# uclanlp/visualbert

Measured on NVIDIA H100. Metric: image-text pairs/sec fwd+bwd VisualBERT-base, higher is better.
Workload: dtype bf16

## Files before the change

### visualbert_b200/csrc/vb_attention.cuh

```cuda
#pragma once
#include <stdlib.h>

#include "../../include/vbert_b200.h"
#include "vb_common.cuh"

namespace vb {


constexpr int kHd = 64;
constexpr int kBlk = 64;
constexpr int kTileBytes = kBlk * kHd * 2;
constexpr float kLog2e = 1.4426950408889634f;

struct AttnParams {
    const bf16* qkv;
    const float* mask_bias;
    bf16* ctx;
    float* lse;
    const bf16* dctx;
    bf16* dqkv;
    float* drow;
    unsigned long long* keep;
    int B, S, A, H;
    float scale;
// ... 190 lines not shown
#pragma unroll
    for (int nt = 0; nt < 8; ++nt) m |= static_cast<unsigned long long>((bits16 >> (2 * nt)) & 3u) << (nt * 8 + 2 * t);
    m |= __shfl_xor_sync(0xffffffffu, m, 1);
    m |= __shfl_xor_sync(0xffffffffu, m, 2);
    return m;
}
__device__ __forceinline__ void store_acc(bf16* base, long long ld, int row0, int nrows, const float (&c)[8][4],
                                          int lane, float mul0, float mul1) {
    const int g = lane >> 2, t = lane & 3;
    const int ra = row0 + g, rb = row0 + g + 8;
#pragma unroll
    for (int nt = 0; nt < 8; ++nt) {
        const int col = nt * 8 + 2 * t;
        if (ra < nrows)
            *reinterpret_cast<uint32_t*>(base + static_cast<long long>(ra) * ld + col) =
                pack_bf16x2(c[nt][0] * mul0, c[nt][1] * mul0);
        if (rb < nrows)
            *reinterpret_cast<uint32_t*>(base + static_cast<long long>(rb) * ld + col) =
                pack_bf16x2(c[nt][2] * mul1, c[nt][3] * mul1);
    }
}


constexpr int kMaxSub = 4;

int attn_fwd_head(const AttnParams& p, int nkb, cudaStream_t st, bool mask_ready);
int attn_bwd_head(const AttnParams& p, int nkb, cudaStream_t st, bool delta_ready);
int attn_keep_mask(const AttnParams& p, int nkb, cudaStream_t st);
int attn_delta(const AttnParams& p, cudaStream_t st);
bool attn_wgmma_supported(const AttnParams& p);
int attn_fwd_wgmma(const AttnParams& p, cudaStream_t st, bool mask_ready);
int attn_bwd_wgmma(const AttnParams& p, cudaStream_t st, bool delta_ready);
int make_tmap_bf16(CUtensorMap* m, const void* ptr, uint64_t inner, uint64_t outer, uint64_t ld_elems, uint32_t box_outer);

}
```

### visualbert_b200/csrc/vb_attention_wgmma.cu

```cuda
#include "vb_attention.cuh"

namespace vb {

constexpr int kWgTile = kBlk * kHd * 2;
constexpr int kMaxWgmmaBlocks = 3;

template <int NKB>
struct AttnSmem {
    static constexpr int FWD_BYTES = 3 * NKB * kWgTile + NKB * kBlk * 4 + 16 + 1024;
    static constexpr int BWD_BYTES = (4 * NKB + NKB * NKB) * kWgTile + NKB * kBlk * 4 + 16 + 1024;
};

__device__ __forceinline__ uint64_t tile_desc(uint32_t saddr) { return wgmma_desc_sw128(saddr, kWgTile, 1024); }

__device__ __forceinline__ unsigned long long keep_word(const AttnParams& p, unsigned bh, int q, int kb, int nkb, int t) {
    if (p.drop_scale == 0.f) return ~0ull;
    return p.keep[(static_cast<unsigned long long>(bh) * (nkb * kBlk) + q) * nkb + kb] >> (2 * t);
}

template <int NKB>
__device__ __forceinline__ void qk_block(float (&s)[32], uint32_t sQ, uint32_t sK, int wg, int kb) {
#pragma unroll
    for (int k = 0; k < kHd / 16; ++k)
        wgmma_m64n64k16_ss<0, 0>(s, tile_desc(sQ + wg * kWgTile + k * 32), tile_desc(sK + kb * kWgTile + k * 32), k > 0 ? 1u : 0u);
}
__device__ __forceinline__ void pack_afrag(uint32_t (&a)[4], const float (&x)[32], int kk) {
    a[0] = pack_bf16x2(x[8 * kk], x[8 * kk + 1]);
    a[1] = pack_bf16x2(x[8 * kk + 2], x[8 * kk + 3]);
    a[2] = pack_bf16x2(x[8 * kk + 4], x[8 * kk + 5]);
    a[3] = pack_bf16x2(x[8 * kk + 6], x[8 * kk + 7]);
}
__device__ __forceinline__ void store_rows(bf16* base, long long ld, int r0, int nrows, const float (&x)[32], int t, float mul0, float mul1) {
#pragma unroll
    for (int j = 0; j < 8; ++j) {
        const int col = 8 * j + 2 * t;
        if (r0 < nrows) *reinterpret_cast<uint32_t*>(base + static_cast<long long>(r0) * ld + col) = pack_bf16x2(x[4 * j] * mul0, x[4 * j + 1] * mul0);
        if (r0 + 8 < nrows)
            *reinterpret_cast<uint32_t*>(base + static_cast<long long>(r0 + 8) * ld + col) = pack_bf16x2(x[4 * j + 2] * mul1, x[4 * j + 3] * mul1);
    }
}
__device__ __forceinline__ void store_tile(uint32_t tile, int r, const float (&x)[32], int t) {
#pragma unroll
    for (int j = 0; j < 8; ++j) {
        st_shared_u32(tile + swz(r, j) + 4 * t, pack_bf16x2(x[4 * j], x[4 * j + 1]));
        st_shared_u32(tile + swz(r + 8, j) + 4 * t, pack_bf16x2(x[4 * j + 2], x[4 * j + 3]));
    }
}

template <int NKB>
__global__ void __launch_bounds__(NKB * 128, 1)
attn_fwd_wgmma_kernel(const __grid_constant__ CUtensorMap tmQKV, const AttnParams p) {
    extern __shared__ uint8_t smem_raw[];
    const uint32_t raw = smem_u32(smem_raw);
    const uint32_t base = (raw + 1023u) & ~1023u;
    uint8_t* smem = smem_raw + (base - raw);
    const uint32_t sQ = base, sK = base + NKB * kWgTile, sV = base + 2 * NKB * kWgTile;
    float* sbias = reinterpret_cast<float*>(smem + 3 * NKB * kWgTile);
    const uint32_t bar = base + 3 * NKB * kWgTile + NKB * kBlk * 4;
    const int tid = threadIdx.x, wg = tid >> 7, warp = (tid >> 5) & 3, lane = tid & 31, g = lane >> 2, t = lane & 3;
    const int item = blockIdx.x, b = item / p.A, h = item % p.A, S = p.S;
    const unsigned bh = static_cast<unsigned>(item);

    if (tid == 0) {
        tma_prefetch_desc(&tmQKV);
        mbar_init(bar, 1);
        fence_barrier_init();
    }
    __syncthreads();
    pdl_trigger();
    pdl_wait();
    if (tid == 0) {
        mbar_arrive_expect_tx(bar, 3 * NKB * kWgTile);
#pragma unroll
        for (int m = 0; m < 3; ++m)
#pragma unroll
            for (int kb = 0; kb < NKB; ++kb) tma_load_2d(base + (m * NKB + kb) * kWgTile, &tmQKV, bar, m * p.H + h * kHd, b * S + kb * kBlk);
    }
    for (int i = tid; i < NKB * kBlk; i += NKB * 128) sbias[i] = i < S ? p.mask_bias[static_cast<long long>(b) * S + i] * kLog2e : -INFINITY;
    const int q0 = wg * kBlk + warp * 16 + g;
    unsigned long long keep[NKB][2];
#pragma unroll
    for (int kb = 0; kb < NKB; ++kb) {
        keep[kb][0] = keep_word(p, bh, q0, kb, NKB, t);
        keep[kb][1] = keep_word(p, bh, q0 + 8, kb, NKB, t);
    }
    __syncthreads();
    mbar_wait(bar, 0);

    float s[NKB][32];
    wgmma_fence();
#pragma unroll
    for (int kb = 0; kb < NKB; ++kb) qk_block<NKB>(s[kb], sQ, sK, wg, kb);
    wgmma_commit();
    wgmma_wait<0>();

    const float sc2 = p.scale * kLog2e;
    float mx[2] = {-INFINITY, -INFINITY};
#pragma unroll
    for (int kb = 0; kb < NKB; ++kb)
#pragma unroll
        for (int j = 0; j < 8; ++j) {
            const float b0 = sbias[kb * kBlk + 8 * j + 2 * t], b1 = sbias[kb * kBlk + 8 * j + 2 * t + 1];
            s[kb][4 * j] = fmaf(s[kb][4 * j], sc2, b0); s[kb][4 * j + 1] = fmaf(s[kb][4 * j + 1], sc2, b1);
            s[kb][4 * j + 2] = fmaf(s[kb][4 * j + 2], sc2, b0); s[kb][4 * j + 3] = fmaf(s[kb][4 * j + 3], sc2, b1);
            mx[0] = fmaxf(mx[0], fmaxf(s[kb][4 * j], s[kb][4 * j + 1]));
            mx[1] = fmaxf(mx[1], fmaxf(s[kb][4 * j + 2], s[kb][4 * j + 3]));
        }
    float l[2] = {0.f, 0.f};
#pragma unroll
    for (int r = 0; r < 2; ++r) {
        mx[r] = fmaxf(mx[r], __shfl_xor_sync(0xffffffffu, mx[r], 1));
        mx[r] = fmaxf(mx[r], __shfl_xor_sync(0xffffffffu, mx[r], 2));
    }
#pragma unroll
    for (int kb = 0; kb < NKB; ++kb)
#pragma unroll
        for (int j = 0; j < 8; ++j)
#pragma unroll
            for (int c = 0; c < 4; ++c) {
                const int r = c >> 1;
                float e = fast_ex2(s[kb][4 * j + c] - mx[r]);
                l[r] += e;
                if (!((keep[kb][r] >> (8 * j + (c & 1))) & 1ull)) e = 0.f;
                s[kb][4 * j + c] = e;
            }
#pragma unroll
    for (int r = 0; r < 2; ++r) {
        l[r] += __shfl_xor_sync(0xffffffffu, l[r], 1);
        l[r] += __shfl_xor_sync(0xffffffffu, l[r], 2);
    }

    uint32_t pa[NKB][4][4];
#pragma unroll
    for (int kb = 0; kb < NKB; ++kb)
#pragma unroll
        for (int kk = 0; kk < 4; ++kk) pack_afrag(pa[kb][kk], s[kb], kk);
    float o[32];
    wgmma_fence();
#pragma unroll
    for (int kb = 0; kb < NKB; ++kb)
#pragma unroll
        for (int kk = 0; kk < 4; ++kk)
            wgmma_m64n64k16_rs<1>(o, pa[kb][kk], tile_desc(sV + kb * kWgTile + kk * 2048), (kb > 0 || kk > 0) ? 1u : 0u);
    wgmma_commit();
    wgmma_wait<0>();

    const float dscale = p.drop_scale != 0.f ? p.drop_scale : 1.f;
    store_rows(p.ctx + static_cast<long long>(b) * S * p.H + h * kHd, p.H, q0, S, o, t, dscale / l[0], dscale / l[1]);
    if (t == 0 && p.lse != nullptr) {
        float* lse = p.lse + static_cast<long long>(item) * S;
        if (q0 < S) lse[q0] = (mx[0] + log2f(l[0])) * 0.6931471805599453f;
        if (q0 + 8 < S) lse[q0 + 8] = (mx[1] + log2f(l[1])) * 0.6931471805599453f;
    }
}

template <int NKB>
__global__ void __launch_bounds__(NKB * 128, 1)
attn_bwd_wgmma_kernel(const __grid_constant__ CUtensorMap tmQKV, const __grid_constant__ CUtensorMap tmDO, const AttnParams p) {
    extern __shared__ uint8_t smem_raw[];
    const uint32_t raw = smem_u32(smem_raw);
    const uint32_t base = (raw + 1023u) & ~1023u;
    uint8_t* smem = smem_raw + (base - raw);
    const uint32_t sQ = base, sK = base + NKB * kWgTile, sV = base + 2 * NKB * kWgTile, sDO = base + 3 * NKB * kWgTile;
    const uint32_t sPS = base + 4 * NKB * kWgTile;
    float* sbias = reinterpret_cast<float*>(smem + (4 * NKB + NKB * NKB) * kWgTile);
    const uint32_t bar = base + (4 * NKB + NKB * NKB) * kWgTile + NKB * kBlk * 4;
    const int tid = threadIdx.x, wg = tid >> 7, warp = (tid >> 5) & 3, lane = tid & 31, g = lane >> 2, t = lane & 3;
    const int item = blockIdx.x, b = item / p.A, h = item % p.A, S = p.S;
    const unsigned bh = static_cast<unsigned>(item);
    const long long ld = 3LL * p.H;

    if (tid == 0) {
        tma_prefetch_desc(&tmQKV);
        tma_prefetch_desc(&tmDO);
        mbar_init(bar, 1);
        fence_barrier_init();
    }
    __syncthreads();
    pdl_trigger();
    pdl_wait();
    if (tid == 0) {
        mbar_arrive_expect_tx(bar, 4 * NKB * kWgTile);
#pragma unroll
        for (int kb = 0; kb < NKB; ++kb) {
#pragma unroll
            for (int m = 0; m < 3; ++m) tma_load_2d(base + (m * NKB + kb) * kWgTile, &tmQKV, bar, m * p.H + h * kHd, b * S + kb * kBlk);
            tma_load_2d(sDO + kb * kWgTile, &tmDO, bar, h * kHd, b * S + kb * kBlk);
        }
    }
    for (int i = tid; i < NKB * kBlk; i += NKB * 128) sbias[i] = i < S ? p.mask_bias[static_cast<long long>(b) * S + i] * kLog2e : -INFINITY;
    const int r0 = warp * 16 + g;
    const int q0 = wg * kBlk + r0;
    float lse2[2], dr[2];
#pragma unroll
    for (int r = 0; r < 2; ++r) {
        const int q = q0 + 8 * r;
        lse2[r] = q < S ? p.lse[static_cast<long long>(item) * S + q] * kLog2e : INFINITY;
        dr[r] = q < S ? p.drow[static_cast<long long>(item) * S + q] : 0.f;
    }
    unsigned long long keep[NKB][2];
#pragma unroll
    for (int kb = 0; kb < NKB; ++kb) {
        keep[kb][0] = keep_word(p, bh, q0, kb, NKB, t);
        keep[kb][1] = keep_word(p, bh, q0 + 8, kb, NKB, t);
    }
    __syncthreads();
    mbar_wait(bar, 0);
    const float sc2 = p.scale * kLog2e;
    const float ds = p.drop_scale != 0.f ? p.drop_scale : 1.f;
    auto probs = [&](float (&s)[32], int kb) {
#pragma unroll
        for (int j = 0; j < 8; ++j)
#pragma unroll
            for (int c = 0; c < 4; ++c)
                s[4 * j + c] = fast_ex2(fmaf(s[4 * j + c], sc2, sbias[kb * kBlk + 8 * j + 2 * t + (c & 1)]) - lse2[c >> 1]);
    };
    auto kept = [&](int kb, int j, int c) { return ((keep[kb][c >> 1] >> (8 * j + (c & 1))) & 1ull) != 0; };
    bf16* dqkv = p.dqkv + static_cast<long long>(b) * S * ld + h * kHd;

#pragma unroll
    for (int kb = 0; kb < NKB; ++kb) {
        float s[32];
        wgmma_fence();
        qk_block<NKB>(s, sQ, sK, wg, kb);
        wgmma_commit();
        wgmma_wait<0>();
        probs(s, kb);
#pragma unroll
        for (int j = 0; j < 8; ++j)
#pragma unroll
            for (int c = 0; c < 4; ++c) s[4 * j + c] = kept(kb, j, c) ? s[4 * j + c] * ds : 0.f;
        store_tile(sPS + (wg * NKB + kb) * kWgTile, r0, s, t);
    }
    fence_proxy_async_smem();
    __syncthreads();
    {
        float acc[32];
        wgmma_fence();
#pragma unroll
        for (int qb = 0; qb < NKB; ++qb)
#pragma unroll
            for (int kk = 0; kk < 4; ++kk)
                wgmma_m64n64k16_ss<1, 1>(acc, tile_desc(sPS + (qb * NKB + wg) * kWgTile + kk * 2048), tile_desc(sDO + qb * kWgTile + kk * 2048),
                                         (qb > 0 || kk > 0) ? 1u : 0u);
        wgmma_commit();
        wgmma_wait<0>();
        store_rows(dqkv + 2 * p.H, ld, q0, S, acc, t, 1.f, 1.f);
    }
    __syncthreads();

    float dq[32];
#pragma unroll
    for (int kb = 0; kb < NKB; ++kb) {
        float s[32], dp[32];
        wgmma_fence();
        qk_block<NKB>(s, sQ, sK, wg, kb);
#pragma unroll
        for (int k = 0; k < kHd / 16; ++k)
            wgmma_m64n64k16_ss<0, 0>(dp, tile_desc(sDO + wg * kWgTile + k * 32), tile_desc(sV + kb * kWgTile + k * 32), k > 0 ? 1u : 0u);
        wgmma_commit();
        wgmma_wait<0>();
        probs(s, kb);
#pragma unroll
        for (int j = 0; j < 8; ++j)
#pragma unroll
            for (int c = 0; c < 4; ++c) {
                const float dpd = kept(kb, j, c) ? dp[4 * j + c] * ds : 0.f;
                s[4 * j + c] *= dpd - dr[c >> 1];
            }
        store_tile(sPS + (wg * NKB + kb) * kWgTile, r0, s, t);
        uint32_t pa[4][4];
#pragma unroll
        for (int kk = 0; kk < 4; ++kk) pack_afrag(pa[kk], s, kk);
        wgmma_fence();
#pragma unroll
        for (int kk = 0; kk < 4; ++kk)
            wgmma_m64n64k16_rs<1>(dq, pa[kk], tile_desc(sK + kb * kWgTile + kk * 2048), (kb > 0 || kk > 0) ? 1u : 0u);
        wgmma_commit();
        wgmma_wait<0>();
    }
    store_rows(dqkv, ld, q0, S, dq, t, p.scale, p.scale);
    fence_proxy_async_smem();
    __syncthreads();
    {
        float acc[32];
        wgmma_fence();
#pragma unroll
        for (int qb = 0; qb < NKB; ++qb)
#pragma unroll
            for (int kk = 0; kk < 4; ++kk)
                wgmma_m64n64k16_ss<1, 1>(acc, tile_desc(sPS + (qb * NKB + wg) * kWgTile + kk * 2048), tile_desc(sQ + qb * kWgTile + kk * 2048),
                                         (qb > 0 || kk > 0) ? 1u : 0u);
        wgmma_commit();
        wgmma_wait<0>();
        store_rows(dqkv + p.H, ld, q0, S, acc, t, p.scale, p.scale);
    }
}

bool attn_wgmma_supported(const AttnParams& p) {
    return p.S <= kMaxWgmmaBlocks * kBlk && (reinterpret_cast<uintptr_t>(p.qkv) & 15) == 0 && (p.H * 2) % 16 == 0 &&
           (p.dctx == nullptr || (reinterpret_cast<uintptr_t>(p.dctx) & 15) == 0);
}

template <int NKB>
static int launch_fwd_wgmma(const AttnParams& p, const CUtensorMap& tq, cudaStream_t st) {
    auto kern = attn_fwd_wgmma_kernel<NKB>;
    static int configured[kMaxDevices] = {0};
    VB_CHECK_CUDA(ensure_dyn_smem(kern, AttnSmem<NKB>::FWD_BYTES, configured));
    ProfScope ps(st, PROF_ATTN_FWD, 4.0 * p.B * p.A * p.S * p.S * kHd, 1);
    VB_CHECK_CUDA(launch_pdl(kern, dim3(p.B * p.A), dim3(NKB * 128), AttnSmem<NKB>::FWD_BYTES, st, tq, p));
    return 0;
}
template <int NKB>
static int launch_bwd_wgmma(const AttnParams& p, const CUtensorMap& tq, const CUtensorMap& td, cudaStream_t st) {
    auto kern = attn_bwd_wgmma_kernel<NKB>;
    static int configured[kMaxDevices] = {0};
    VB_CHECK_CUDA(ensure_dyn_smem(kern, AttnSmem<NKB>::BWD_BYTES, configured));
    ProfScope ps(st, PROF_ATTN_DKV, 10.0 * p.B * p.A * p.S * p.S * kHd, 1);
    VB_CHECK_CUDA(launch_pdl(kern, dim3(p.B * p.A), dim3(NKB * 128), AttnSmem<NKB>::BWD_BYTES, st, tq, td, p));
    return 0;
}

int attn_fwd_wgmma(const AttnParams& p, cudaStream_t st, bool mask_ready) {
    const int nkb = (p.S + kBlk - 1) / kBlk;
    if (!mask_ready) {
        int rc = attn_keep_mask(p, nkb, st);
        if (rc) return rc;
    }
    CUtensorMap tq;
    int rc = make_tmap_bf16(&tq, p.qkv, 3ull * p.H, static_cast<uint64_t>(p.B) * p.S, 3ull * p.H, kBlk);
    if (rc) return rc;
    if (nkb == 1) rc = launch_fwd_wgmma<1>(p, tq, st);
    else if (nkb == 2) rc = launch_fwd_wgmma<2>(p, tq, st);
    else rc = launch_fwd_wgmma<3>(p, tq, st);
    if (rc) return rc;
    VB_CHECK_CUDA(cudaGetLastError());
    return 0;
}

int attn_bwd_wgmma(const AttnParams& p, cudaStream_t st, bool delta_ready) {
    const int nkb = (p.S + kBlk - 1) / kBlk;
    int rc = 0;
    if (!delta_ready) {
        rc = attn_delta(p, st);
        if (rc) return rc;
    }
    CUtensorMap tq, td;
    rc = make_tmap_bf16(&tq, p.qkv, 3ull * p.H, static_cast<uint64_t>(p.B) * p.S, 3ull * p.H, kBlk);
    if (rc) return rc;
    rc = make_tmap_bf16(&td, p.dctx, static_cast<uint64_t>(p.H), static_cast<uint64_t>(p.B) * p.S, static_cast<uint64_t>(p.H), kBlk);
    if (rc) return rc;
    if (nkb == 1) rc = launch_bwd_wgmma<1>(p, tq, td, st);
    else if (nkb == 2) rc = launch_bwd_wgmma<2>(p, tq, td, st);
    else rc = launch_bwd_wgmma<3>(p, tq, td, st);
    if (rc) return rc;
    VB_CHECK_CUDA(cudaGetLastError());
    return 0;
}

}
```

### visualbert_b200/csrc/vb_common.cuh

```cuda
#pragma once

#include <cuda.h>
#include <cuda_bf16.h>
#include <cuda_runtime.h>
#include <stdint.h>
#include <stdio.h>

#include <atomic>

namespace vb {

typedef __nv_bfloat16 bf16;

extern std::atomic<long long> g_launches;
int num_sms();
constexpr int kMaxDevices = 64;
int current_device();
template <typename K>
inline cudaError_t ensure_dyn_smem(K kern, int bytes, int (&cache)[kMaxDevices]) {
    const int d = current_device();
    if (cache[d] >= bytes) return cudaSuccess;
    cudaError_t e = cudaFuncSetAttribute(kern, cudaFuncAttributeMaxDynamicSharedMemorySize, bytes);
    if (e == cudaSuccess) cache[d] = bytes;
    return e;
// ... 156 lines not shown
__device__ __forceinline__ bool mbar_try_wait(uint32_t bar, uint32_t parity) {
    uint32_t ok;
    asm volatile(
        "{\n"
        ".reg .pred p;\n"
        "mbarrier.try_wait.parity.shared::cta.b64 p, [%1], %2;\n"
        "selp.u32 %0, 1, 0, p;\n"
        "}\n"
        : "=r"(ok)
        : "r"(bar), "r"(parity)
        : "memory");
    return ok != 0;
}
__device__ __forceinline__ void mbar_wait(uint32_t bar, uint32_t parity) {
    if (mbar_try_wait(bar, parity)) return;
    const long long t0 = clock64();
    uint32_t spins = 0;
    while (!mbar_try_wait(bar, parity)) {
        if ((++spins & 0x3ffu) == 0 && clock64() - t0 > 4000000000ll) __trap();
    }
}

__device__ __forceinline__ void tma_prefetch_desc(const CUtensorMap* m) {
    asm volatile("prefetch.tensormap [%0];" ::"l"(reinterpret_cast<uint64_t>(m)) : "memory");
}
__device__ __forceinline__ void tma_load_2d(uint32_t smem_dst, const CUtensorMap* m, uint32_t bar,
                                            int c_inner, int c_outer) {
    asm volatile(
        "cp.async.bulk.tensor.2d.shared::cluster.global.mbarrier::complete_tx::bytes"
        " [%0], [%1, {%3, %4}], [%2];"
        ::"r"(smem_dst), "l"(reinterpret_cast<uint64_t>(m)), "r"(bar), "r"(c_inner), "r"(c_outer)
        : "memory");
}

__device__ __forceinline__ uint64_t wgmma_desc_sw128(uint32_t saddr, uint32_t lbo_bytes, uint32_t sbo_bytes) {
    return static_cast<uint64_t>((saddr & 0x3FFFFu) >> 4) | (static_cast<uint64_t>((lbo_bytes >> 4) & 0x3FFFu) << 16) |
           (static_cast<uint64_t>((sbo_bytes >> 4) & 0x3FFFu) << 32) | (1ull << 62);
}
__device__ __forceinline__ void wgmma_fence() { asm volatile("wgmma.fence.sync.aligned;" ::: "memory"); }
__device__ __forceinline__ void wgmma_commit() { asm volatile("wgmma.commit_group.sync.aligned;" ::: "memory"); }
template <int N>
__device__ __forceinline__ void wgmma_wait() { asm volatile("wgmma.wait_group.sync.aligned %0;" ::"n"(N) : "memory"); }
template <int TA, int TB>
__device__ __forceinline__ void wgmma_m64n128k16(float (&d)[64], uint64_t a_desc, uint64_t b_desc, uint32_t accumulate) {
    asm volatile(
        "{\n"
        ".reg .pred p;\n"
        "setp.ne.b32 p, %66, 0;\n"
        "wgmma.mma_async.sync.aligned.m64n128k16.f32.bf16.bf16 "
        "{%0, %1, %2, %3, %4, %5, %6, %7, %8, %9, %10, %11, %12, %13, %14, %15, %16, %17, %18, %19, %20, %21, %22, %23, %24, %25, %26, %27, %28, %29, %30, %31, %32, %33, %34, %35, %36, %37, %38, %39, %40, %41, %42, %43, %44, %45, %46, %47, %48, %49, %50, %51, %52, %53, %54, %55, %56, %57, %58, %59, %60, %61, %62, %63}, "
        "%64, %65, p, 1, 1, %67, %68;\n"
        "}\n"
        : "+f"(d[0]), "+f"(d[1]), "+f"(d[2]), "+f"(d[3]), "+f"(d[4]), "+f"(d[5]), "+f"(d[6]), "+f"(d[7]),
          "+f"(d[8]), "+f"(d[9]), "+f"(d[10]), "+f"(d[11]), "+f"(d[12]), "+f"(d[13]), "+f"(d[14]), "+f"(d[15]),
          "+f"(d[16]), "+f"(d[17]), "+f"(d[18]), "+f"(d[19]), "+f"(d[20]), "+f"(d[21]), "+f"(d[22]), "+f"(d[23]),
          "+f"(d[24]), "+f"(d[25]), "+f"(d[26]), "+f"(d[27]), "+f"(d[28]), "+f"(d[29]), "+f"(d[30]), "+f"(d[31]),
          "+f"(d[32]), "+f"(d[33]), "+f"(d[34]), "+f"(d[35]), "+f"(d[36]), "+f"(d[37]), "+f"(d[38]), "+f"(d[39]),
          "+f"(d[40]), "+f"(d[41]), "+f"(d[42]), "+f"(d[43]), "+f"(d[44]), "+f"(d[45]), "+f"(d[46]), "+f"(d[47]),
          "+f"(d[48]), "+f"(d[49]), "+f"(d[50]), "+f"(d[51]), "+f"(d[52]), "+f"(d[53]), "+f"(d[54]), "+f"(d[55]),
          "+f"(d[56]), "+f"(d[57]), "+f"(d[58]), "+f"(d[59]), "+f"(d[60]), "+f"(d[61]), "+f"(d[62]), "+f"(d[63])
        : "l"(a_desc), "l"(b_desc), "r"(accumulate), "n"(TA), "n"(TB));
}
template <int TA, int TB>
__device__ __forceinline__ void wgmma_m64n64k16_ss(float (&d)[32], uint64_t a_desc, uint64_t b_desc, uint32_t accumulate) {
    asm volatile(
        "{\n"
// ... 67 lines not shown
```

### visualbert_b200/csrc/vb_gemm.cu

```cuda
#include <stdarg.h>
#include <stdio.h>
#include <stdlib.h>
#include <string.h>

#include <atomic>
#include <mutex>
#include <vector>

#include "../../include/vbert_b200.h"
#include "vb_common.cuh"

namespace vb {

static thread_local char g_err[1024] = "";
std::atomic<long long> g_launches{0};

void set_error(const char* fmt, ...) {
    va_list ap;
    va_start(ap, fmt);
    vsnprintf(g_err, sizeof(g_err), fmt, ap);
    va_end(ap);
}
const char* get_error() { return g_err; }

// ... 399 lines not shown
                              const cuuint32_t* box) {
    TmapKey k;
    memset(&k, 0, sizeof(k));
    k.ptr = ptr; k.rank = rank; k.dev = current_device();
    k.d0 = dims[0]; k.d1 = dims[1]; k.d2 = rank > 2 ? dims[2] : 1;
    k.s0 = strides[0]; k.s1 = rank > 2 ? strides[1] : 0;
    k.b0 = box[0]; k.b1 = box[1]; k.b2 = rank > 2 ? box[2] : 1;
    uint64_t h = reinterpret_cast<uintptr_t>(ptr) * 0x9E3779B97F4A7C15ull;
    h ^= (k.d0 * 31 + k.d1) * 0xBF58476D1CE4E5B9ull + k.d2 * 1315423911ull + k.s0 * 2654435761ull + k.s1 * 40503ull;
    h ^= (static_cast<uint64_t>(k.b1) << 20) ^ (static_cast<uint64_t>(k.b0) << 8) ^ k.b2 ^ (static_cast<uint64_t>(k.dev) << 40);
    h ^= h >> 29;
    if (g_tmap_cache == nullptr) { g_tmap_cache = new std::vector<TmapSlot>(kTmapSlots); for (auto& sl : *g_tmap_cache) sl.used = false; }
    TmapSlot& sl = (*g_tmap_cache)[h & (kTmapSlots - 1)];
    if (sl.used && sl.key == k) { *m = sl.map; return 0; }
    EncodeTiledFn fn = get_encode_fn();
    VB_REQUIRE(fn != nullptr, "cuTensorMapEncodeTiled unavailable (driver too old / no GPU?)");
    cuuint32_t estr[3] = {1, 1, 1};
    CUresult r = fn(m, CU_TENSOR_MAP_DATA_TYPE_BFLOAT16, rank, const_cast<void*>(ptr), dims, strides, box, estr,
                    CU_TENSOR_MAP_INTERLEAVE_NONE, CU_TENSOR_MAP_SWIZZLE_128B, CU_TENSOR_MAP_L2_PROMOTION_L2_256B,
                    CU_TENSOR_MAP_FLOAT_OOB_FILL_NONE);
    VB_REQUIRE(r == CUDA_SUCCESS, "cuTensorMapEncodeTiled (rank %u) failed with CUresult %d", rank, static_cast<int>(r));
    sl.key = k; sl.map = *m; sl.used = true;
    return 0;
}

int make_tmap_bf16(CUtensorMap* m, const void* ptr, uint64_t inner, uint64_t outer, uint64_t ld_elems,
                   uint32_t box_outer) {
    VB_REQUIRE((reinterpret_cast<uintptr_t>(ptr) & 15) == 0, "TMA operand not 16-byte aligned");
    VB_REQUIRE((ld_elems * 2) % 16 == 0, "TMA operand row stride must be a multiple of 8 elements");
    cuuint64_t dims[2] = {inner, outer};
    cuuint64_t strides[1] = {ld_elems * 2};
    cuuint32_t box[2] = {64, box_outer};
    return encode_tmap_cached(m, ptr, 2, dims, strides, box);
}

int current_device() {
    int dev = 0;
    cudaGetDevice(&dev);
    return (dev < 0 || dev >= kMaxDevices) ? 0 : dev;
}

int num_sms() {
    static int n[kMaxDevices] = {0};
    const int dev = current_device();
    if (n[dev] == 0) {
        int v = 0;
        cudaDeviceGetAttribute(&v, cudaDevAttrMultiProcessorCount, dev);
        n[dev] = v > 0 ? v : 132;
    }
    return n[dev];
}

template <bool A_MN, bool B_MN, int BLOCK_N, bool OUT_F32, int EPI = EPI_GENERIC>
static int launch(const CUtensorMap& ta, const CUtensorMap& tb, const GemmParams& p, cudaStream_t st) {
    using C = Cfg<BLOCK_N>;
    auto kern = gemm_wgmma_kernel<A_MN, B_MN, BLOCK_N, OUT_F32, EPI>;
    static int configured[kMaxDevices] = {0};
    VB_CHECK_CUDA(ensure_dyn_smem(kern, C::SMEM_BYTES, configured));
    const long long tiles = static_cast<long long>((p.M + BLOCK_M - 1) / BLOCK_M) * ((p.N + BLOCK_N - 1) / BLOCK_N) * p.splits;
    VB_REQUIRE(tiles < (1LL << 31), "vb_gemm: too many tiles");
    {
        ProfScope ps(st, OUT_F32 ? PROF_GEMM_WGRAD : (B_MN ? PROF_GEMM_DGRAD : PROF_GEMM_FWD), 2.0 * p.M * p.N * p.K, 1);
        VB_CHECK_CUDA(launch_pdl(kern, dim3(static_cast<unsigned>(tiles)), dim3(kThreads), C::SMEM_BYTES, st, ta, tb, p));
    }
    VB_CHECK_CUDA(cudaGetLastError());
    return 0;
// ... 167 lines not shown
```

Measured before the change: 3029.

## Make attention fwd/bwd kernels persistent with double-buffered TMA prefetch of next head

Attention forward and backward kernels become persistent: the grid is capped at SMs times occupancy and each block loops over (batch, head) items. While the current item computes, the next item's Q/K/V (forward) or Q/dO (backward) tiles are prefetched into a second shared-memory stage, along with its bias, LSE and dropout words. K/V in backward are reloaded after their last use. A 3D tensor map (inner, rows, batch) replaces the 2D one, so out-of-range rows are zero-filled per batch instead of reading into the next sequence. The cost is double the shared memory for staging, which may lower occupancy or block larger NKB configs.

Result: no change. 3042 (median of 6 runs) (+0.4%).

```diff
diff --git a/visualbert_b200/csrc/vb_attention.cuh b/visualbert_b200/csrc/vb_attention.cuh
--- a/visualbert_b200/csrc/vb_attention.cuh
+++ b/visualbert_b200/csrc/vb_attention.cuh
@@ -246,5 +246,7 @@
 int attn_fwd_wgmma(const AttnParams& p, cudaStream_t st, bool mask_ready);
 int attn_bwd_wgmma(const AttnParams& p, cudaStream_t st, bool delta_ready);
 int make_tmap_bf16(CUtensorMap* m, const void* ptr, uint64_t inner, uint64_t outer, uint64_t ld_elems, uint32_t box_outer);
-
-}
+int make_tmap_bf16_3d(CUtensorMap* m, const void* ptr, uint64_t inner, uint64_t rows, uint64_t batches, uint64_t ld_elems,
+                      uint32_t box_rows);
+
+}
diff --git a/visualbert_b200/csrc/vb_attention_wgmma.cu b/visualbert_b200/csrc/vb_attention_wgmma.cu
--- a/visualbert_b200/csrc/vb_attention_wgmma.cu
+++ b/visualbert_b200/csrc/vb_attention_wgmma.cu
@@ -7,8 +7,8 @@
 
 template <int NKB>
 struct AttnSmem {
-    static constexpr int FWD_BYTES = 3 * NKB * kWgTile + NKB * kBlk * 4 + 16 + 1024;
-    static constexpr int BWD_BYTES = (4 * NKB + NKB * NKB) * kWgTile + NKB * kBlk * 4 + 16 + 1024;
+    static constexpr int FWD_BYTES = 2 * 3 * NKB * kWgTile + 2 * NKB * kBlk * 4 + 16 + 1024;
+    static constexpr int BWD_BYTES = (6 * NKB + NKB * NKB) * kWgTile + NKB * kBlk * 4 + 32 + 1024;
 };
 
 __device__ __forceinline__ uint64_t tile_desc(uint32_t saddr) { return wgmma_desc_sw128(saddr, kWgTile, 1024); }
@@ -46,111 +46,131 @@
         st_shared_u32(tile + swz(r + 8, j) + 4 * t, pack_bf16x2(x[4 * j + 2], x[4 * j + 3]));
     }
 }
+template <int NKB>
+__device__ __forceinline__ void load_bias(float* sbias, const AttnParams& p, int b, int tid) {
+    for (int i = tid; i < NKB * kBlk; i += NKB * 128) sbias[i] = i < p.S ? p.mask_bias[static_cast<long long>(b) * p.S + i] * kLog2e : -INFINITY;
+}
 
 template <int NKB>
 __global__ void __launch_bounds__(NKB * 128, 1)
 attn_fwd_wgmma_kernel(const __grid_constant__ CUtensorMap tmQKV, const AttnParams p) {
+    constexpr int kStage = 3 * NKB * kWgTile;
     extern __shared__ uint8_t smem_raw[];
     const uint32_t raw = smem_u32(smem_raw);
     const uint32_t base = (raw + 1023u) & ~1023u;
     uint8_t* smem = smem_raw + (base - raw);
-    const uint32_t sQ = base, sK = base + NKB * kWgTile, sV = base + 2 * NKB * kWgTile;
-    float* sbias = reinterpret_cast<float*>(smem + 3 * NKB * kWgTile);
-    const uint32_t bar = base + 3 * NKB * kWgTile + NKB * kBlk * 4;
+    float* sbias0 = reinterpret_cast<float*>(smem + 2 * kStage);
+    const uint32_t bar0 = base + 2 * kStage + 2 * NKB * kBlk * 4;
     const int tid = threadIdx.x, wg = tid >> 7, warp = (tid >> 5) & 3, lane = tid & 31, g = lane >> 2, t = lane & 3;
-    const int item = blockIdx.x, b = item / p.A, h = item % p.A, S = p.S;
-    const unsigned bh = static_cast<unsigned>(item);
+    const int S = p.S, total = p.B * p.A;
+    const int q0 = wg * kBlk + warp * 16 + g;
+
+    auto load_item = [&](int it, int st) {
+        const int b = it / p.A, h = it % p.A;
+        const uint32_t bar = bar0 + 8 * st;
+        mbar_arrive_expect_tx(bar, kStage);
+#pragma unroll
+        for (int m = 0; m < 3; ++m)
+#pragma unroll
+            for (int kb = 0; kb < NKB; ++kb)
+                tma_load_3d(base + st * kStage + (m * NKB + kb) * kWgTile, &tmQKV, bar, m * p.H + (h * kHd), kb * kBlk, b);
+    };
+    unsigned long long keep[NKB][2];
+    auto read_item = [&](int it, int st) {
+        load_bias<NKB>(sbias0 + st * NKB * kBlk, p, it / p.A, tid);
+#pragma unroll
+        for (int kb = 0; kb < NKB; ++kb) {
+            keep[kb][0] = keep_word(p, static_cast<unsigned>(it), q0, kb, NKB, t);
+            keep[kb][1] = keep_word(p, static_cast<unsigned>(it), q0 + 8, kb, NKB, t);
+        }
+    };
 
     if (tid == 0) {
         tma_prefetch_desc(&tmQKV);
-        mbar_init(bar, 1);
+        mbar_init(bar0, 1);
+        mbar_init(bar0 + 8, 1);
         fence_barrier_init();
     }
     __syncthreads();
     pdl_trigger();
     pdl_wait();
-    if (tid == 0) {
-        mbar_arrive_expect_tx(bar, 3 * NKB * kWgTile);
-#pragma unroll
-        for (int m = 0; m < 3; ++m)
-#pragma unroll
-            for (int kb = 0; kb < NKB; ++kb) tma_load_2d(base + (m * NKB + kb) * kWgTile, &tmQKV, bar, m * p.H + h * kHd, b * S + kb * kBlk);
-    }
-    for (int i = tid; i < NKB * kBlk; i += NKB * 128) sbias[i] = i < S ? p.mask_bias[static_cast<long long>(b) * S + i] * kLog2e : -INFINITY;
-    const int q0 = wg * kBlk + warp * 16 + g;
-    unsigned long long keep[NKB][2];
-#pragma unroll
-    for (int kb = 0; kb < NKB; ++kb) {
-        keep[kb][0] = keep_word(p, bh, q0, kb, NKB, t);
-        keep[kb][1] = keep_word(p, bh, q0 + 8, kb, NKB, t);
-    }
-    __syncthreads();
-    mbar_wait(bar, 0);
-
-    float s[NKB][32];
-    wgmma_fence();
-#pragma unroll
-    for (int kb = 0; kb < NKB; ++kb) qk_block<NKB>(s[kb], sQ, sK, wg, kb);
-    wgmma_commit();
-    wgmma_wait<0>();
-
-    const float sc2 = p.scale * kLog2e;
-    float mx[2] = {-INFINITY, -INFINITY};
-#pragma unroll
-    for (int kb = 0; kb < NKB; ++kb)
-#pragma unroll
-        for (int j = 0; j < 8; ++j) {
-            const float b0 = sbias[kb * kBlk + 8 * j + 2 * t], b1 = sbias[kb * kBlk + 8 * j + 2 * t + 1];
-            s[kb][4 * j] = fmaf(s[kb][4 * j], sc2, b0); s[kb][4 * j + 1] = fmaf(s[kb][4 * j + 1], sc2, b1);
-            s[kb][4 * j + 2] = fmaf(s[kb][4 * j + 2], sc2, b0); s[kb][4 * j + 3] = fmaf(s[kb][4 * j + 3], sc2, b1);
-            mx[0] = fmaxf(mx[0], fmaxf(s[kb][4 * j], s[kb][4 * j + 1]));
-            mx[1] = fmaxf(mx[1], fmaxf(s[kb][4 * j + 2], s[kb][4 * j + 3]));
-        }
-    float l[2] = {0.f, 0.f};
-#pragma unroll
-    for (int r = 0; r < 2; ++r) {
-        mx[r] = fmaxf(mx[r], __shfl_xor_sync(0xffffffffu, mx[r], 1));
-        mx[r] = fmaxf(mx[r], __shfl_xor_sync(0xffffffffu, mx[r], 2));
-    }
-#pragma unroll
-    for (int kb = 0; kb < NKB; ++kb)
-#pragma unroll
-        for (int j = 0; j < 8; ++j)
-#pragma unroll
-            for (int c = 0; c < 4; ++c) {
-                const int r = c >> 1;
-                float e = fast_ex2(s[kb][4 * j + c] - mx[r]);
-                l[r] += e;
-                if (!((keep[kb][r] >> (8 * j + (c & 1))) & 1ull)) e = 0.f;
-                s[kb][4 * j + c] = e;
+    if (tid == 0) load_item(blockIdx.x, 0);
+    read_item(blockIdx.x, 0);
+
+    for (int item = blockIdx.x, i = 0; item < total; item += gridDim.x, ++i) {
+        const int st = i & 1, b = item / p.A, h = item % p.A, next = item + gridDim.x;
+        const uint32_t sQ = base + st * kStage, sK = sQ + NKB * kWgTile, sV = sQ + 2 * NKB * kWgTile;
+        const float* sbias = sbias0 + st * NKB * kBlk;
+        __syncthreads();
+        if (tid == 0 && next < total) load_item(next, st ^ 1);
+        mbar_wait(bar0 + 8 * st, (i >> 1) & 1);
+
+        float s[NKB][32];
+        wgmma_fence();
+#pragma unroll
+        for (int kb = 0; kb < NKB; ++kb) qk_block<NKB>(s[kb], sQ, sK, wg, kb);
+        wgmma_commit();
+        wgmma_wait<0>();
+
+        const float sc2 = p.scale * kLog2e;
+        float mx[2] = {-INFINITY, -INFINITY};
+#pragma unroll
+        for (int kb = 0; kb < NKB; ++kb)
+#pragma unroll
+            for (int j = 0; j < 8; ++j) {
+                const float b0 = sbias[kb * kBlk + 8 * j + 2 * t], b1 = sbias[kb * kBlk + 8 * j + 2 * t + 1];
+                s[kb][4 * j] = fmaf(s[kb][4 * j], sc2, b0); s[kb][4 * j + 1] = fmaf(s[kb][4 * j + 1], sc2, b1);
+                s[kb][4 * j + 2] = fmaf(s[kb][4 * j + 2], sc2, b0); s[kb][4 * j + 3] = fmaf(s[kb][4 * j + 3], sc2, b1);
+                mx[0] = fmaxf(mx[0], fmaxf(s[kb][4 * j], s[kb][4 * j + 1]));
+                mx[1] = fmaxf(mx[1], fmaxf(s[kb][4 * j + 2], s[kb][4 * j + 3]));
             }
-#pragma unroll
-    for (int r = 0; r < 2; ++r) {
-        l[r] += __shfl_xor_sync(0xffffffffu, l[r], 1);
-        l[r] += __shfl_xor_sync(0xffffffffu, l[r], 2);
-    }
-
-    uint32_t pa[NKB][4][4];
-#pragma unroll
-    for (int kb = 0; kb < NKB; ++kb)
-#pragma unroll
-        for (int kk = 0; kk < 4; ++kk) pack_afrag(pa[kb][kk], s[kb], kk);
-    float o[32];
-    wgmma_fence();
-#pragma unroll
-    for (int kb = 0; kb < NKB; ++kb)
-#pragma unroll
-        for (int kk = 0; kk < 4; ++kk)
-            wgmma_m64n64k16_rs<1>(o, pa[kb][kk], tile_desc(sV + kb * kWgTile + kk * 2048), (kb > 0 || kk > 0) ? 1u : 0u);
-    wgmma_commit();
-    wgmma_wait<0>();
-
-    const float dscale = p.drop_scale != 0.f ? p.drop_scale : 1.f;
-    store_rows(p.ctx + static_cast<long long>(b) * S * p.H + h * kHd, p.H, q0, S, o, t, dscale / l[0], dscale / l[1]);
-    if (t == 0 && p.lse != nullptr) {
-        float* lse = p.lse + static_cast<long long>(item) * S;
-        if (q0 < S) lse[q0] = (mx[0] + log2f(l[0])) * 0.6931471805599453f;
-        if (q0 + 8 < S) lse[q0 + 8] = (mx[1] + log2f(l[1])) * 0.6931471805599453f;
+        float l[2] = {0.f, 0.f};
+#pragma unroll
+        for (int r = 0; r < 2; ++r) {
+            mx[r] = fmaxf(mx[r], __shfl_xor_sync(0xffffffffu, mx[r], 1));
+            mx[r] = fmaxf(mx[r], __shfl_xor_sync(0xffffffffu, mx[r], 2));
+        }
+#pragma unroll
+        for (int kb = 0; kb < NKB; ++kb)
+#pragma unroll
+            for (int j = 0; j < 8; ++j)
+#pragma unroll
+                for (int c = 0; c < 4; ++c) {
+                    const int r = c >> 1;
+                    float e = fast_ex2(s[kb][4 * j + c] - mx[r]);
+                    l[r] += e;
+                    if (!((keep[kb][r] >> (8 * j + (c & 1))) & 1ull)) e = 0.f;
+                    s[kb][4 * j + c] = e;
+                }
+#pragma unroll
+        for (int r = 0; r < 2; ++r) {
+            l[r] += __shfl_xor_sync(0xffffffffu, l[r], 1);
+            l[r] += __shfl_xor_sync(0xffffffffu, l[r], 2);
+        }
+
+        uint32_t pa[NKB][4][4];
+#pragma unroll
+        for (int kb = 0; kb < NKB; ++kb)
+#pragma unroll
+            for (int kk = 0; kk < 4; ++kk) pack_afrag(pa[kb][kk], s[kb], kk);
+        float o[32];
+        wgmma_fence();
+#pragma unroll
+        for (int kb = 0; kb < NKB; ++kb)
+#pragma unroll
+            for (int kk = 0; kk < 4; ++kk)
+                wgmma_m64n64k16_rs<1>(o, pa[kb][kk], tile_desc(sV + kb * kWgTile + kk * 2048), (kb > 0 || kk > 0) ? 1u : 0u);
+        wgmma_commit();
+        if (next < total) read_item(next, st ^ 1);
+        wgmma_wait<0>();
+
+        const float dscale = p.drop_scale != 0.f ? p.drop_scale : 1.f;
+        store_rows(p.ctx + static_cast<long long>(b) * S * p.H + h * kHd, p.H, q0, S, o, t, dscale / l[0], dscale / l[1]);
+        if (t == 0 && p.lse != nullptr) {
+            float* lse = p.lse + static_cast<long long>(item) * S;
+            if (q0 < S) lse[q0] = (mx[0] + log2f(l[0])) * 0.6931471805599453f;
+            if (q0 + 8 < S) lse[q0 + 8] = (mx[1] + log2f(l[1])) * 0.6931471805599453f;
+        }
     }
 }
 
@@ -161,51 +181,71 @@
     const uint32_t raw = smem_u32(smem_raw);
     const uint32_t base = (raw + 1023u) & ~1023u;
     uint8_t* smem = smem_raw + (base - raw);
-    const uint32_t sQ = base, sK = base + NKB * kWgTile, sV = base + 2 * NKB * kWgTile, sDO = base + 3 * NKB * kWgTile;
-    const uint32_t sPS = base + 4 * NKB * kWgTile;
-    float* sbias = reinterpret_cast<float*>(smem + (4 * NKB + NKB * NKB) * kWgTile);
-    const uint32_t bar = base + (4 * NKB + NKB * NKB) * kWgTile + NKB * kBlk * 4;
+    const uint32_t sQ0 = base, sDO0 = base + 2 * NKB * kWgTile, sK = base + 4 * NKB * kWgTile, sV = base + 5 * NKB * kWgTile;
+    const uint32_t sPS = base + 6 * NKB * kWgTile;
+    float* sbias = reinterpret_cast<float*>(smem + (6 * NKB + NKB * NKB) * kWgTile);
+    const uint32_t barQD0 = base + (6 * NKB + NKB * NKB) * kWgTile + NKB * kBlk * 4;
+    const uint32_t barK = barQD0 + 16, barV = barQD0 + 24;
     const int tid = threadIdx.x, wg = tid >> 7, warp = (tid >> 5) & 3, lane = tid & 31, g = lane >> 2, t = lane & 3;
-    const int item = blockIdx.x, b = item / p.A, h = item % p.A, S = p.S;
-    const unsigned bh = static_cast<unsigned>(item);
+    const int S = p.S, total = p.B * p.A;
     const long long ld = 3LL * p.H;
+    const int r0 = warp * 16 + g;
+    const int q0 = wg * kBlk + r0;
+
+    auto load_qdo = [&](int it, int s) {
+        const int b = it / p.A, h = it % p.A;
+        const uint32_t bar = barQD0 + 8 * s;
+        mbar_arrive_expect_tx(bar, 2 * NKB * kWgTile);
+#pragma unroll
+        for (int kb = 0; kb < NKB; ++kb) {
+            tma_load_3d(sQ0 + (s * NKB + kb) * kWgTile, &tmQKV, bar, h * kHd, kb * kBlk, b);
+            tma_load_3d(sDO0 + (s * NKB + kb) * kWgTile, &tmDO, bar, h * kHd, kb * kBlk, b);
+        }
+    };
+    auto load_kv = [&](int it) {
+        const int b = it / p.A, h = it % p.A;
+        mbar_arrive_expect_tx(barK, NKB * kWgTile);
+#pragma unroll
+        for (int kb = 0; kb < NKB; ++kb) tma_load_3d(sK + kb * kWgTile, &tmQKV, barK, p.H + h * kHd, kb * kBlk, b);
+        mbar_arrive_expect_tx(barV, NKB * kWgTile);
+#pragma unroll
+        for (int kb = 0; kb < NKB; ++kb) tma_load_3d(sV + kb * kWgTile, &tmQKV, barV, 2 * p.H + h * kHd, kb * kBlk, b);
+    };
+    float lse2[2], dr[2];
+    unsigned long long keep[NKB][2];
+    auto read_item = [&](int it) {
+        load_bias<NKB>(sbias, p, it / p.A, tid);
+#pragma unroll
+        for (int r = 0; r < 2; ++r) {
+            const int q = q0 + 8 * r;
+            lse2[r] = q < S ? p.lse[static_cast<long long>(it) * S + q] * kLog2e : INFINITY;
+            dr[r] = q < S ? p.drow[static_cast<long long>(it) * S + q] : 0.f;
+        }
+#pragma unroll
+        for (int kb = 0; kb < NKB; ++kb) {
+            keep[kb][0] = keep_word(p, static_cast<unsigned>(it), q0, kb, NKB, t);
+            keep[kb][1] = keep_word(p, static_cast<unsigned>(it), q0 + 8, kb, NKB, t);
+        }
+    };
 
     if (tid == 0) {
         tma_prefetch_desc(&tmQKV);
         tma_prefetch_desc(&tmDO);
-        mbar_init(bar, 1);
+        mbar_init(barQD0, 1);
+        mbar_init(barQD0 + 8, 1);
+        mbar_init(barK, 1);
+        mbar_init(barV, 1);
         fence_barrier_init();
     }
     __syncthreads();
     pdl_trigger();
     pdl_wait();
     if (tid == 0) {
-        mbar_arrive_expect_tx(bar, 4 * NKB * kWgTile);
-#pragma unroll
-        for (int kb = 0; kb < NKB; ++kb) {
-#pragma unroll
-            for (int m = 0; m < 3; ++m) tma_load_2d(base + (m * NKB + kb) * kWgTile, &tmQKV, bar, m * p.H + h * kHd, b * S + kb * kBlk);
-            tma_load_2d(sDO + kb * kWgTile, &tmDO, bar, h * kHd, b * S + kb * kBlk);
-        }
-    }
-    for (int i = tid; i < NKB * kBlk; i += NKB * 128) sbias[i] = i < S ? p.mask_bias[static_cast<long long>(b) * S + i] * kLog2e : -INFINITY;
-    const int r0 = warp * 16 + g;
-    const int q0 = wg * kBlk + r0;
-    float lse2[2], dr[2];
-#pragma unroll
-    for (int r = 0; r < 2; ++r) {
-        const int q = q0 + 8 * r;
-        lse2[r] = q < S ? p.lse[static_cast<long long>(item) * S + q] * kLog2e : INFINITY;
-        dr[r] = q < S ? p.drow[static_cast<long long>(item) * S + q] : 0.f;
-    }
-    unsigned long long keep[NKB][2];
-#pragma unroll
-    for (int kb = 0; kb < NKB; ++kb) {
-        keep[kb][0] = keep_word(p, bh, q0, kb, NKB, t);
-        keep[kb][1] = keep_word(p, bh, q0 + 8, kb, NKB, t);
-    }
-    __syncthreads();
-    mbar_wait(bar, 0);
+        load_qdo(blockIdx.x, 0);
+        load_kv(blockIdx.x);
+    }
+    read_item(blockIdx.x);
+
     const float sc2 = p.scale * kLog2e;
     const float ds = p.drop_scale != 0.f ? p.drop_scale : 1.f;
     auto probs = [&](float (&s)[32], int kb) {
@@ -216,84 +256,97 @@
                 s[4 * j + c] = fast_ex2(fmaf(s[4 * j + c], sc2, sbias[kb * kBlk + 8 * j + 2 * t + (c & 1)]) - lse2[c >> 1]);
     };
     auto kept = [&](int kb, int j, int c) { return ((keep[kb][c >> 1] >> (8 * j + (c & 1))) & 1ull) != 0; };
-    bf16* dqkv = p.dqkv + static_cast<long long>(b) * S * ld + h * kHd;
-
-#pragma unroll
-    for (int kb = 0; kb < NKB; ++kb) {
-        float s[32];
-        wgmma_fence();
-        qk_block<NKB>(s, sQ, sK, wg, kb);
-        wgmma_commit();
-        wgmma_wait<0>();
-        probs(s, kb);
-#pragma unroll
-        for (int j = 0; j < 8; ++j)
-#pragma unroll
-            for (int c = 0; c < 4; ++c) s[4 * j + c] = kept(kb, j, c) ? s[4 * j + c] * ds : 0.f;
-        store_tile(sPS + (wg * NKB + kb) * kWgTile, r0, s, t);
-    }
-    fence_proxy_async_smem();
-    __syncthreads();
-    {
-        float acc[32];
-        wgmma_fence();
-#pragma unroll
-        for (int qb = 0; qb < NKB; ++qb)
+
+    for (int item = blockIdx.x, i = 0; item < total; item += gridDim.x, ++i) {
+        const int b = item / p.A, h = item % p.A, next = item + gridDim.x;
+        const int slot = i & 1;
+        const uint32_t ph = i & 1, sQ = sQ0 + slot * NKB * kWgTile, sDO = sDO0 + slot * NKB * kWgTile;
+        bf16* dqkv = p.dqkv + static_cast<long long>(b) * S * ld + h * kHd;
+        __syncthreads();
+        if (tid == 0 && next < total) load_qdo(next, slot ^ 1);
+        mbar_wait(barQD0 + 8 * slot, (i >> 1) & 1);
+        mbar_wait(barK, ph);
+
+#pragma unroll
+        for (int kb = 0; kb < NKB; ++kb) {
+            float s[32];
+            wgmma_fence();
+            qk_block<NKB>(s, sQ, sK, wg, kb);
+            wgmma_commit();
+            wgmma_wait<0>();
+            probs(s, kb);
+#pragma unroll
+            for (int j = 0; j < 8; ++j)
+#pragma unroll
+                for (int c = 0; c < 4; ++c) s[4 * j + c] = kept(kb, j, c) ? s[4 * j + c] * ds : 0.f;
+            store_tile(sPS + (wg * NKB + kb) * kWgTile, r0, s, t);
+        }
+        fence_proxy_async_smem();
+        __syncthreads();
+        {
+            float acc[32];
+            wgmma_fence();
+#pragma unroll
+            for (int qb = 0; qb < NKB; ++qb)
+#pragma unroll
+                for (int kk = 0; kk < 4; ++kk)
+                    wgmma_m64n64k16_ss<1, 1>(acc, tile_desc(sPS + (qb * NKB + wg) * kWgTile + kk * 2048), tile_desc(sDO + qb * kWgTile + kk * 2048),
+                                             (qb > 0 || kk > 0) ? 1u : 0u);
+            wgmma_commit();
+            wgmma_wait<0>();
+            store_rows(dqkv + 2 * p.H, ld, q0, S, acc, t, 1.f, 1.f);
+        }
+        __syncthreads();
+        mbar_wait(barV, ph);
+
+        float dq[32];
+#pragma unroll
+        for (int kb = 0; kb < NKB; ++kb) {
+            float s[32], dp[32];
+            wgmma_fence();
+            qk_block<NKB>(s, sQ, sK, wg, kb);
+#pragma unroll
+            for (int k = 0; k < kHd / 16; ++k)
+                wgmma_m64n64k16_ss<0, 0>(dp, tile_desc(sDO + wg * kWgTile + k * 32), tile_desc(sV + kb * kWgTile + k * 32), k > 0 ? 1u : 0u);
+            wgmma_commit();
+            wgmma_wait<0>();
+            probs(s, kb);
+#pragma unroll
+            for (int j = 0; j < 8; ++j)
+#pragma unroll
+                for (int c = 0; c < 4; ++c) {
+                    const float dpd = kept(kb, j, c) ? dp[4 * j + c] * ds : 0.f;
+                    s[4 * j + c] *= dpd - dr[c >> 1];
+                }
+            store_tile(sPS + (wg * NKB + kb) * kWgTile, r0, s, t);
+            uint32_t pa[4][4];
+#pragma unroll
+            for (int kk = 0; kk < 4; ++kk) pack_afrag(pa[kk], s, kk);
+            wgmma_fence();
 #pragma unroll
             for (int kk = 0; kk < 4; ++kk)
-                wgmma_m64n64k16_ss<1, 1>(acc, tile_desc(sPS + (qb * NKB + wg) * kWgTile + kk * 2048), tile_desc(sDO + qb * kWgTile + kk * 2048),
-                                         (qb > 0 || kk > 0) ? 1u : 0u);
-        wgmma_commit();
-        wgmma_wait<0>();
-        store_rows(dqkv + 2 * p.H, ld, q0, S, acc, t, 1.f, 1.f);
-    }
-    __syncthreads();
-
-    float dq[32];
-#pragma unroll
-    for (int kb = 0; kb < NKB; ++kb) {
-        float s[32], dp[32];
-        wgmma_fence();
-        qk_block<NKB>(s, sQ, sK, wg, kb);
-#pragma unroll
-        for (int k = 0; k < kHd / 16; ++k)
-            wgmma_m64n64k16_ss<0, 0>(dp, tile_desc(sDO + wg * kWgTile + k * 32), tile_desc(sV + kb * kWgTile + k * 32), k > 0 ? 1u : 0u);
-        wgmma_commit();
-        wgmma_wait<0>();
-        probs(s, kb);
-#pragma unroll
-        for (int j = 0; j < 8; ++j)
-#pragma unroll
-            for (int c = 0; c < 4; ++c) {
-                const float dpd = kept(kb, j, c) ? dp[4 * j + c] * ds : 0.f;
-                s[4 * j + c] *= dpd - dr[c >> 1];
-            }
-        store_tile(sPS + (wg * NKB + kb) * kWgTile, r0, s, t);
-        uint32_t pa[4][4];
-#pragma unroll
-        for (int kk = 0; kk < 4; ++kk) pack_afrag(pa[kk], s, kk);
-        wgmma_fence();
-#pragma unroll
-        for (int kk = 0; kk < 4; ++kk)
-            wgmma_m64n64k16_rs<1>(dq, pa[kk], tile_desc(sK + kb * kWgTile + kk * 2048), (kb > 0 || kk > 0) ? 1u : 0u);
-        wgmma_commit();
-        wgmma_wait<0>();
-    }
-    store_rows(dqkv, ld, q0, S, dq, t, p.scale, p.scale);
-    fence_proxy_async_smem();
-    __syncthreads();
-    {
-        float acc[32];
-        wgmma_fence();
-#pragma unroll
-        for (int qb = 0; qb < NKB; ++qb)
-#pragma unroll
-            for (int kk = 0; kk < 4; ++kk)
-                wgmma_m64n64k16_ss<1, 1>(acc, tile_desc(sPS + (qb * NKB + wg) * kWgTile + kk * 2048), tile_desc(sQ + qb * kWgTile + kk * 2048),
-                                         (qb > 0 || kk > 0) ? 1u : 0u);
-        wgmma_commit();
-        wgmma_wait<0>();
-        store_rows(dqkv + p.H, ld, q0, S, acc, t, p.scale, p.scale);
+                wgmma_m64n64k16_rs<1>(dq, pa[kk], tile_desc(sK + kb * kWgTile + kk * 2048), (kb > 0 || kk > 0) ? 1u : 0u);
+            wgmma_commit();
+            wgmma_wait<0>();
+        }
+        store_rows(dqkv, ld, q0, S, dq, t, p.scale, p.scale);
+        fence_proxy_async_smem();
+        __syncthreads();
+        if (tid == 0 && next < total) load_kv(next);
+        {
+            float acc[32];
+            wgmma_fence();
+#pragma unroll
+            for (int qb = 0; qb < NKB; ++qb)
+#pragma unroll
+                for (int kk = 0; kk < 4; ++kk)
+                    wgmma_m64n64k16_ss<1, 1>(acc, tile_desc(sPS + (qb * NKB + wg) * kWgTile + kk * 2048), tile_desc(sQ + qb * kWgTile + kk * 2048),
+                                             (qb > 0 || kk > 0) ? 1u : 0u);
+            wgmma_commit();
+            if (next < total) read_item(next);
+            wgmma_wait<0>();
+            store_rows(dqkv + p.H, ld, q0, S, acc, t, p.scale, p.scale);
+        }
     }
 }
 
@@ -302,22 +355,40 @@
            (p.dctx == nullptr || (reinterpret_cast<uintptr_t>(p.dctx) & 15) == 0);
 }
 
+template <typename K>
+static cudaError_t persistent_grid(K kern, int threads, int smem, int items, int (&cache)[kMaxDevices], int* grid) {
+    const int d = current_device();
+    if (cache[d] == 0) {
+        int n = 0;
+        cudaError_t e = cudaOccupancyMaxActiveBlocksPerMultiprocessor(&n, kern, threads, smem);
+        if (e != cudaSuccess) return e;
+        cache[d] = n > 0 ? n : 1;
+    }
+    const long long cap = static_cast<long long>(num_sms()) * cache[d];
+    *grid = items < cap ? items : static_cast<int>(cap);
+    return cudaSuccess;
+}
+
 template <int NKB>
 static int launch_fwd_wgmma(const AttnParams& p, const CUtensorMap& tq, cudaStream_t st) {
     auto kern = attn_fwd_wgmma_kernel<NKB>;
-    static int configured[kMaxDevices] = {0};
+    static int configured[kMaxDevices] = {0}, per_sm[kMaxDevices] = {0};
     VB_CHECK_CUDA(ensure_dyn_smem(kern, AttnSmem<NKB>::FWD_BYTES, configured));
+    int grid = 0;
+    VB_CHECK_CUDA(persistent_grid(kern, NKB * 128, AttnSmem<NKB>::FWD_BYTES, p.B * p.A, per_sm, &grid));
     ProfScope ps(st, PROF_ATTN_FWD, 4.0 * p.B * p.A * p.S * p.S * kHd, 1);
-    VB_CHECK_CUDA(launch_pdl(kern, dim3(p.B * p.A), dim3(NKB * 128), AttnSmem<NKB>::FWD_BYTES, st, tq, p));
+    VB_CHECK_CUDA(launch_pdl(kern, dim3(grid), dim3(NKB * 128), AttnSmem<NKB>::FWD_BYTES, st, tq, p));
     return 0;
 }
 template <int NKB>
 static int launch_bwd_wgmma(const AttnParams& p, const CUtensorMap& tq, const CUtensorMap& td, cudaStream_t st) {
     auto kern = attn_bwd_wgmma_kernel<NKB>;
-    static int configured[kMaxDevices] = {0};
+    static int configured[kMaxDevices] = {0}, per_sm[kMaxDevices] = {0};
     VB_CHECK_CUDA(ensure_dyn_smem(kern, AttnSmem<NKB>::BWD_BYTES, configured));
+    int grid = 0;
+    VB_CHECK_CUDA(persistent_grid(kern, NKB * 128, AttnSmem<NKB>::BWD_BYTES, p.B * p.A, per_sm, &grid));
     ProfScope ps(st, PROF_ATTN_DKV, 10.0 * p.B * p.A * p.S * p.S * kHd, 1);
-    VB_CHECK_CUDA(launch_pdl(kern, dim3(p.B * p.A), dim3(NKB * 128), AttnSmem<NKB>::BWD_BYTES, st, tq, td, p));
+    VB_CHECK_CUDA(launch_pdl(kern, dim3(grid), dim3(NKB * 128), AttnSmem<NKB>::BWD_BYTES, st, tq, td, p));
     return 0;
 }
 
@@ -328,7 +399,7 @@
         if (rc) return rc;
     }
     CUtensorMap tq;
-    int rc = make_tmap_bf16(&tq, p.qkv, 3ull * p.H, static_cast<uint64_t>(p.B) * p.S, 3ull * p.H, kBlk);
+    int rc = make_tmap_bf16_3d(&tq, p.qkv, 3ull * p.H, static_cast<uint64_t>(p.S), static_cast<uint64_t>(p.B), 3ull * p.H, kBlk);
     if (rc) return rc;
     if (nkb == 1) rc = launch_fwd_wgmma<1>(p, tq, st);
     else if (nkb == 2) rc = launch_fwd_wgmma<2>(p, tq, st);
@@ -346,9 +417,10 @@
         if (rc) return rc;
     }
     CUtensorMap tq, td;
-    rc = make_tmap_bf16(&tq, p.qkv, 3ull * p.H, static_cast<uint64_t>(p.B) * p.S, 3ull * p.H, kBlk);
+    rc = make_tmap_bf16_3d(&tq, p.qkv, 3ull * p.H, static_cast<uint64_t>(p.S), static_cast<uint64_t>(p.B), 3ull * p.H, kBlk);
     if (rc) return rc;
-    rc = make_tmap_bf16(&td, p.dctx, static_cast<uint64_t>(p.H), static_cast<uint64_t>(p.B) * p.S, static_cast<uint64_t>(p.H), kBlk);
+    rc = make_tmap_bf16_3d(&td, p.dctx, static_cast<uint64_t>(p.H), static_cast<uint64_t>(p.S), static_cast<uint64_t>(p.B),
+                           static_cast<uint64_t>(p.H), kBlk);
     if (rc) return rc;
     if (nkb == 1) rc = launch_bwd_wgmma<1>(p, tq, td, st);
     else if (nkb == 2) rc = launch_bwd_wgmma<2>(p, tq, td, st);
diff --git a/visualbert_b200/csrc/vb_common.cuh b/visualbert_b200/csrc/vb_common.cuh
--- a/visualbert_b200/csrc/vb_common.cuh
+++ b/visualbert_b200/csrc/vb_common.cuh
@@ -212,6 +212,13 @@
         ::"r"(smem_dst), "l"(reinterpret_cast<uint64_t>(m)), "r"(bar), "r"(c_inner), "r"(c_outer)
         : "memory");
 }
+__device__ __forceinline__ void tma_load_3d(uint32_t smem_dst, const CUtensorMap* m, uint32_t bar, int c0, int c1, int c2) {
+    asm volatile(
+        "cp.async.bulk.tensor.3d.shared::cluster.global.mbarrier::complete_tx::bytes"
+        " [%0], [%1, {%3, %4, %5}], [%2];"
+        ::"r"(smem_dst), "l"(reinterpret_cast<uint64_t>(m)), "r"(bar), "r"(c0), "r"(c1), "r"(c2)
+        : "memory");
+}
 
 __device__ __forceinline__ uint64_t wgmma_desc_sw128(uint32_t saddr, uint32_t lbo_bytes, uint32_t sbo_bytes) {
     return static_cast<uint64_t>((saddr & 0x3FFFFu) >> 4) | (static_cast<uint64_t>((lbo_bytes >> 4) & 0x3FFFu) << 16) |
diff --git a/visualbert_b200/csrc/vb_gemm.cu b/visualbert_b200/csrc/vb_gemm.cu
--- a/visualbert_b200/csrc/vb_gemm.cu
+++ b/visualbert_b200/csrc/vb_gemm.cu
@@ -455,6 +455,16 @@
     cuuint64_t strides[1] = {ld_elems * 2};
     cuuint32_t box[2] = {64, box_outer};
     return encode_tmap_cached(m, ptr, 2, dims, strides, box);
+}
+
+int make_tmap_bf16_3d(CUtensorMap* m, const void* ptr, uint64_t inner, uint64_t rows, uint64_t batches, uint64_t ld_elems,
+                      uint32_t box_rows) {
+    VB_REQUIRE((reinterpret_cast<uintptr_t>(ptr) & 15) == 0, "TMA operand not 16-byte aligned");
+    VB_REQUIRE((ld_elems * 2) % 16 == 0, "TMA operand row stride must be a multiple of 8 elements");
+    cuuint64_t dims[3] = {inner, rows, batches};
+    cuuint64_t strides[2] = {ld_elems * 2, rows * ld_elems * 2};
+    cuuint32_t box[3] = {64, box_rows, 1};
+    return encode_tmap_cached(m, ptr, 3, dims, strides, box);
 }
 
 int current_device() {
```
